# anisanazim/Movie-Recommendation-Engine

Measured on AMD Instinct MI355X. Metric: item embeddings/sec + top-K ANN queries/sec, ML-25M d=256, 1/2/4/8 GPU, higher is better.
Workload: dtype f64 cdf / f32 features / fp4 sign planes (exact integer Hamming); 1 GPU; SYN-25M (ML-25M-shaped: U=162541 M=59047 R=25000095), F=128 H=256 d=256, 2 GCN layers, W=100 L=2 T=10, LSH 512-bit, 10000 queries K=11, rng=numpy (the reference's np.random MT19937 stream generated on device: neighbour ids bit-exact with the reference CPU path); global_items=59047, queries=10000, parallelism=item-shard x1

## Files before the change

movie-recommendation-engine_amd/csrc/mt19937.hip:

```cpp
#include "ps_common.h"

#ifndef PS_MT_DEBUG
#define PS_MT_DEBUG 0
#endif

namespace {

constexpr int MT_N = 624, MT_M = 397;
constexpr int DEG = 19937;
constexpr int CHUNK_LOG2 = 17;
constexpr int64_t CHUNK = (int64_t)1 << CHUNK_LOG2;

struct WinSet { int n; long long first[4]; long long cum[5]; };
struct Wanted { int n; long long lo[4], hi[4]; };
__host__ __device__ __forceinline__ long long win_of(const WinSet &ws, long long q) {
    long long w = ws.first[0] + q;
#pragma unroll
    for (int i = 1; i < 4; ++i)
        if (i < ws.n && q >= ws.cum[i]) w = ws.first[i] + (q - ws.cum[i]);
    return w;
}

__device__ __forceinline__ uint32_t twist(uint32_t u, uint32_t v) {
    const uint32_t y = (u & 0x80000000u) | (v & 0x7fffffffu);
    return (y >> 1) ^ ((v & 1u) ? 0x9908b0dfu : 0u);
}
__device__ __forceinline__ uint32_t temper(uint32_t y) {
    y ^= (y >> 11);
    y ^= (y << 7) & 0x9d2c5680u;
    y ^= (y << 15) & 0xefc60000u;
    y ^= (y >> 18);
    return y;
}

__device__ __forceinline__ void next_block(const uint32_t *o, uint32_t *n, int t) {
    if (t < 227) {
        const uint32_t a = o[t + MT_M] ^ twist(o[t], o[t + 1]);
        const uint32_t b = a ^ twist(o[227 + t], o[228 + t]);
        n[t] = a;
        n[227 + t] = b;
        if (t < 169) n[454 + t] = b ^ twist(o[454 + t], o[455 + t]);
        else if (t == 169) n[623] = b ^ twist(o[623], o[MT_M] ^ twist(o[0], o[1]));
    }
    __syncthreads();
}

template <typename Emit>
__device__ __forceinline__ void next_block_emit(const uint32_t *o, uint32_t *n, int t, Emit emit) {
    if (t < 227) {
        const int t3 = t < 169 ? 454 + t : 622;
        const uint32_t x0 = o[t], x1 = o[t + 1], xm = o[t + MT_M], y0 = o[227 + t], y1 = o[228 + t], z0 = o[t3], z1 = o[t3 + 1];
        const uint32_t l623 = o[623], lm = o[MT_M], l0 = o[0], l1 = o[1];
        const uint32_t a = xm ^ twist(x0, x1);
        const uint32_t b = a ^ twist(y0, y1);
        const uint32_t c = b ^ (t < 169 ? twist(z0, z1) : twist(l623, lm ^ twist(l0, l1)));
        n[t] = a;
        n[227 + t] = b;
        emit(t, a);
        emit(227 + t, b);
        if (t <= 169) {
            const int i3 = t < 169 ? 454 + t : 623;
            n[i3] = c;
            emit(i3, c);
        }
    }
    if (!(PS_MT_DEBUG & 32)) __syncthreads();
}

__device__ __forceinline__ uint32_t untwist(uint32_t tmp) {
    const uint32_t m = (uint32_t)((int32_t)tmp >> 31);
    return __builtin_amdgcn_alignbit(tmp ^ (m & 0x9908b0dfu), tmp, 31);
}

template <typename Emit>
__device__ __forceinline__ void prev_block_emit(const uint32_t *o, uint32_t *p, int t, Emit emit) {
    constexpr uint32_t UP = 0x80000000u, LO = 0x7fffffffu;
    if (t < 227) {
        const int tm = t > 0 ? t - 1 : 0, u = t < 170 ? t : 169;
        const uint32_t a0 = o[t + 395], a1 = o[t + 396], a2 = o[t + 397], b0 = o[t + 168], b1 = o[t + 169], b2 = o[t + 170];
        const uint32_t c0 = o[tm], c1 = o[t], d0 = o[226 + u], d1 = o[227 + u], l622 = o[622], l623 = o[623];
        const uint32_t y397 = untwist(a2 ^ b2), y396 = untwist(a1 ^ b1), y395 = untwist(a0 ^ b0);
        const uint32_t n397 = (y397 & UP) | (y396 & LO);
        const uint32_t n396 = (y396 & UP) | (y395 & LO);
        uint32_t n623 = 0;
        if (t == 0) n623 = (untwist(l623 ^ a1) & UP) | (untwist(l622 ^ a0) & LO);
        const uint32_t ylo = untwist((t > 0 ? c0 : n623) ^ n396);
        const uint32_t nt = (untwist(c1 ^ n397) & UP) | (ylo & LO);
        p[t] = nt;
        p[t + 397] = n397;
        emit(t, nt);
        emit(t + 397, n397);
        if (t < 170) {
            const uint32_t v = (untwist(d1 ^ c1) & UP) | (untwist(d0 ^ (t > 0 ? c0 : n623)) & LO);
            p[227 + t] = v;
            emit(227 + t, v);
        }
    }
    if (!(PS_MT_DEBUG & 32)) __syncthreads();
}

__global__ __launch_bounds__(256) void mt_words_kernel(const uint32_t *state_in, int pos_in, int64_t nwords,
                                                       uint32_t *raw, uint32_t *state_out, int32_t *pos_out) {
    __shared__ uint32_t mt[2][MT_N];
    const int t = threadIdx.x;
    for (int i = t; i < MT_N; i += 256) mt[0][i] = state_in[i];
    __syncthreads();
    int cur = 0, pos = pos_in;
    int64_t done = 0;
    while (done < nwords) {
        if (pos >= MT_N) {
            next_block(mt[cur], mt[cur ^ 1], t);
            cur ^= 1;
            pos = 0;
        }
        const int64_t rem = nwords - done;
        const int take = (MT_N - pos) < rem ? (MT_N - pos) : (int)rem;
        for (int i = t; i < take; i += 256) raw[done + i] = temper(mt[cur][pos + i]);
        pos += take;
        done += take;
    }
    __syncthreads();
    for (int i = t; i < MT_N; i += 256) state_out[i] = mt[cur][i];
    if (t == 0) pos_out[0] = pos;
}

__global__ void mt_pairs_to_double_kernel(double *out, int64_t n) {
    for (int64_t i = (int64_t)blockIdx.x * blockDim.x + threadIdx.x; i < n; i += (int64_t)gridDim.x * blockDim.x) {
        const uint2 w = reinterpret_cast<const uint2 *>(out)[i];
        out[i] = ((double)(w.x >> 5) * 67108864.0 + (double)(w.y >> 6)) * (1.0 / 9007199254740992.0);
    }
}

__global__ __launch_bounds__(256) void mt_prepare_kernel(const uint32_t *state_in, int pos_in, uint32_t *w1,
                                                         uint32_t *word0) {
    __shared__ uint32_t seq[3 * MT_N];
    const int t = threadIdx.x;
    for (int i = t; i < MT_N; i += 256) seq[i] = state_in[i];
    __syncthreads();
    next_block(seq, seq + MT_N, t);
    next_block(seq + MT_N, seq + 2 * MT_N, t);
    for (int i = t; i < MT_N; i += 256) w1[i] = seq[pos_in + 1 + i];
    if (t == 0) word0[0] = seq[pos_in];
}

constexpr int JP = 24;
constexpr int PW = MT_N / JP;
constexpr int SEQ_PAD = 34 * MT_N;
constexpr int XB = 17;
static_assert(SEQ_PAD >= DEG + MT_N && JP * PW == MT_N, "jump geometry");

__device__ __forceinline__ uint32_t load_window_word(const uint32_t *parts, int nparts, int t) {
    uint32_t v = 0;
    for (int p = 0; p < nparts; ++p) v ^= parts[p * MT_N + t];
    return v;
}

__global__ __launch_bounds__(256) void mt_expand_kernel(const uint32_t *src, int nparts, int64_t src_stride, uint32_t *seq) {
    __shared__ uint32_t mt[2][MT_N];
    const int t = threadIdx.x;
    uint32_t *out = seq + (size_t)blockIdx.x * SEQ_PAD;
    for (int i = t; i < MT_N; i += 256) {
        const uint32_t v = load_window_word(src + (size_t)blockIdx.x * src_stride, nparts, i);
        mt[0][i] = v;
        out[i] = v;
    }
    __syncthreads();
    int cur = 0;
    for (int blk = 1; blk < 34; ++blk) {
        uint32_t *dst = out + blk * MT_N;
        next_block_emit(mt[cur], mt[cur ^ 1], t, [&](int i, uint32_t v) { dst[i] = v; });
        cur ^= 1;
    }
}

constexpr int CT = MT_N / 4;
__device__ __forceinline__ void combine_part(const uint32_t *s, const uint32_t *poly_part, uint32_t *dst) {
    __shared__ uint32_t sq[PW * 32 + MT_N + 8];
    __shared__ uint32_t pl[PW];
    const int t = threadIdx.x;
    for (int i = t; i < PW * 32 + MT_N; i += 192) sq[i] = s[i];
    if (t < PW) pl[t] = poly_part[t];
    __syncthreads();
    if (t < CT) {
        uint32_t a0 = 0, a1 = 0, a2 = 0, a3 = 0;
        for (int w = 0; w < PW; ++w) {
            uint32_t bits = pl[w];
            const uint32_t *p = sq + w * 32 + t;
            while (bits) {
                uint32_t v[2][4];
#pragma unroll
                for (int u = 0; u < 2; ++u) {
                    const bool on = bits != 0u;
                    const int bu = on ? __builtin_ctz(bits) : 0;
                    v[u][0] = on ? p[bu] : 0u;
                    v[u][1] = on ? p[bu + CT] : 0u;
                    v[u][2] = on ? p[bu + 2 * CT] : 0u;
                    v[u][3] = on ? p[bu + 3 * CT] : 0u;
                    bits &= bits - 1u;
                }
                a0 ^= v[0][0] ^ v[1][0];
                a1 ^= v[0][1] ^ v[1][1];
                a2 ^= v[0][2] ^ v[1][2];
                a3 ^= v[0][3] ^ v[1][3];
            }
        }
        dst[t] = a0;
        dst[t + CT] = a1;
        dst[t + 2 * CT] = a2;
        dst[t + 3 * CT] = a3;
    }
}

__global__ __launch_bounds__(192) void mt_combine_kernel(const uint32_t *seq, const uint32_t *poly, uint32_t *dst_parts) {
    const int b = blockIdx.x / JP, part = blockIdx.x % JP;
    combine_part(seq + (size_t)b * SEQ_PAD + part * PW * 32, poly + part * PW, dst_parts + ((size_t)b * JP + part) * MT_N);
}

__global__ __launch_bounds__(192) void mt_combine_radix_kernel(const uint32_t *seq, const uint32_t *polys, uint32_t *states,
                                                               int64_t have, int64_t K) {
    const int b = blockIdx.x / JP, part = blockIdx.x % JP;
    const int64_t tgt = (int64_t)(blockIdx.y + 1) * have + b;
    if (tgt >= K) return;
    combine_part(seq + (size_t)b * SEQ_PAD + part * PW * 32, polys + (size_t)blockIdx.y * MT_N + part * PW,
                 states + ((size_t)tgt * JP + part) * MT_N);
}

typedef int v4i_t __attribute__((ext_vector_type(4)));
typedef int v8i_t __attribute__((ext_vector_type(8)));
typedef float v16f_t __attribute__((ext_vector_type(16)));

constexpr int KS_TOTAL = 320;
constexpr int PLW = SEQ_PAD / 32;
constexpr int JT = 20, JG = 10;
constexpr int MF_PLANES = 2;
static_assert(SEQ_PAD % 32 == 0 && JT * 32 >= MT_N && JT == 2 * JG && 32 % MF_PLANES == 0, "plane geometry: two waves x JG lag tiles");

__device__ __forceinline__ uint32_t bits_to_fp4(uint32_t byte) {
    auto four = [](uint32_t n) { return (n | (n << 3) | (n << 6) | (n << 9)) & 0x1111u; };
    return (four(byte & 15u) | (four((byte >> 4) & 15u) << 16)) << 1;
}

__global__ __launch_bounds__(256) void mt_pack_polys_kernel(const uint32_t *__restrict__ polys, int rows, uint4 *__restrict__ polyA) {
    const int idx = blockIdx.x * 256 + threadIdx.x;
    if (idx >= KS_TOTAL * 64) return;
    const int ks = idx >> 6, lane = idx & 63, m = lane & 31, w = 2 * ks + (lane >> 5);
    const uint32_t word = (m < rows && w < MT_N) ? polys[(size_t)m * MT_N + w] : 0u;
    polyA[idx] = make_uint4(bits_to_fp4(word & 255u), bits_to_fp4((word >> 8) & 255u), bits_to_fp4((word >> 16) & 255u),
                            bits_to_fp4(word >> 24));
}

__global__ __launch_bounds__(256) void mt_begin_kernel(const uint32_t *__restrict__ state_in, int pos_in, uint32_t *__restrict__ plain0,
                                                       uint32_t *__restrict__ word0, uint32_t *__restrict__ seq,
                                                       const uint32_t *__restrict__ polys, int nrows, int ngroups, uint4 *__restrict__ polyA,
                                                       WinSet ws) {
    const int t = threadIdx.x;
    if (blockIdx.x < 2) {
        const bool back = blockIdx.x == 1;
        __shared__ uint32_t s3[3 * MT_N];
        __shared__ uint32_t mt[2][MT_N];
        if (state_in != nullptr) {
            for (int i = t; i < MT_N; i += 256) s3[i] = state_in[i];
            __syncthreads();
            next_block(s3, s3 + MT_N, t);
            next_block(s3 + MT_N, s3 + 2 * MT_N, t);
        }
        for (int i = t; i < MT_N; i += 256) {
            const uint32_t v = state_in != nullptr ? s3[pos_in + 1 + i] : plain0[i];
            mt[0][i] = v;
            if (!back) {
                if (state_in != nullptr) plain0[i] = v;
                seq[XB * MT_N + i] = v;
            }
        }
        if (t == 0 && !back && state_in != nullptr) word0[0] = s3[pos_in];
        __syncthreads();
        int cur = 0;
        if (!back) {
            for (int blk = XB + 1; blk < 34; ++blk) {
                uint32_t *dst = seq + blk * MT_N;
                next_block_emit(mt[cur], mt[cur ^ 1], t, [&](int i, uint32_t v) { dst[i] = v; });
                cur ^= 1;
            }
        } else {
            for (int blk = XB - 1; blk >= 0; --blk) {
                uint32_t *dst = seq + blk * MT_N;
                prev_block_emit(mt[cur], mt[cur ^ 1], t, [&](int i, uint32_t v) { dst[i] = v; });
                cur ^= 1;
            }
        }
        return;
    }
    const int64_t idx = (int64_t)(blockIdx.x - 2) * 256 + t;
    if (idx >= (int64_t)ngroups * KS_TOTAL * 64) return;
    const int g = (int)(idx / (KS_TOTAL * 64)), rem = (int)(idx % (KS_TOTAL * 64));
    const int ks = rem >> 6, lane = rem & 63, q = 32 * g + (lane & 31), w = 2 * ks + (lane >> 5);
    const uint32_t word = (q < nrows && w < MT_N) ? polys[(size_t)(win_of(ws, q) - 1) * MT_N + w] : 0u;
    polyA[idx] = make_uint4(bits_to_fp4(word & 255u), bits_to_fp4((word >> 8) & 255u), bits_to_fp4((word >> 16) & 255u),
                            bits_to_fp4(word >> 24));
}

__global__ __launch_bounds__(256) void mt_planes_kernel(const uint32_t *__restrict__ seq, uint32_t *__restrict__ planes) {
    const int lane = threadIdx.x & 63, wv = threadIdx.x >> 6;
    const uint32_t *s = seq + (size_t)blockIdx.y * SEQ_PAD;
    uint32_t *pl = planes + (size_t)blockIdx.y * 32 * PLW;
    for (int grp = blockIdx.x * 4 + wv; grp * 64 < SEQ_PAD; grp += gridDim.x * 4) {
        const int i = grp * 64 + lane;
        const uint32_t word = i < SEQ_PAD ? s[i] : 0u;
#pragma unroll
        for (int b = 0; b < 32; ++b) {
            const uint64_t m = __ballot((word >> b) & 1u);
            if (lane == 0) {
                pl[b * PLW + 2 * grp] = (uint32_t)m;
                if (2 * grp + 1 < PLW) pl[b * PLW + 2 * grp + 1] = (uint32_t)(m >> 32);
            }
        }
    }
}

__device__ __forceinline__ v16f_t bit_mfma(const v4i_t &a, const v4i_t &b, const v16f_t &c) {
    const v8i_t A = {a[0], a[1], a[2], a[3], 0, 0, 0, 0};
    const v8i_t B = {b[0], b[1], b[2], b[3], 0, 0, 0, 0};
    return __builtin_amdgcn_mfma_scale_f32_32x32x64_f8f6f4(A, B, c, 4, 4, 0, 0x7f7f7f7f, 0, 0x7f7f7f7f);
}

__global__ __launch_bounds__(256, 2) void mt_jump_mfma_kernel(const uint32_t *__restrict__ planes, const uint4 *__restrict__ polyA,
                                                              uint16_t *__restrict__ PLp, int nsrc, int parts, int steps, int ngroups) {
    extern __shared__ uint32_t copies[];
    const int tid = threadIdx.x, lane = tid & 63, wv = tid >> 6, pb = wv >> 1, g = wv & 1, n = lane & 31, kb = lane >> 5;
    int item = blockIdx.x;
    const int b0 = (item % (32 / MF_PLANES)) * MF_PLANES; item /= (32 / MF_PLANES);
    const int src = item % nsrc, part = item / nsrc;
    const int ks0 = part * steps, J0 = g * JG;
    const int dmin = 2 * ks0;
    const int CW = 4 * (2 * steps + JT + 1) + 8;
    for (int mm = tid; mm < ((PS_MT_DEBUG & 1) ? 64 : MF_PLANES * CW); mm += 256) {
        const int q = mm / CW, m = mm % CW;
        const uint32_t *pl = planes + ((size_t)(src / ngroups) * 32 + b0 + q) * PLW;
        uint32_t *cp = copies + (size_t)q * 8 * CW;
        const int p0 = 32 * dmin + 8 * m;
        const uint32_t w0 = (p0 >> 5) < PLW ? pl[p0 >> 5] : 0u, w1 = ((p0 + 8) >> 5) < PLW ? pl[(p0 + 8) >> 5] : 0u;
        const uint32_t e0 = bits_to_fp4((w0 >> (p0 & 31)) & 255u), e1 = bits_to_fp4((w1 >> ((p0 + 8) & 31)) & 255u);
        cp[m] = e0;
#pragma unroll
        for (int c = 1; c < 8; ++c) cp[c * CW + m] = __builtin_amdgcn_alignbit(e1, e0, 4 * c);
    }
    __syncthreads();
    const int b = b0 + pb;
    const uint32_t *frag = copies + (size_t)pb * 8 * CW + (n & 7) * CW + 4 * (J0 + kb) + (n >> 3);
    auto load_r = [&](int x) { const uint32_t *q = frag + 4 * x; return v4i_t{(int)q[0], (int)q[1], (int)q[2], (int)q[3]}; };
    const uint4 *pa = polyA + ((size_t)(src % ngroups) * KS_TOTAL + ks0) * 64 + lane;
    auto load_a = [&](v4i_t &dst, int u) {
        const uint4 *ptr = pa + (size_t)u * 64;
        asm volatile("global_load_dwordx4 %0, %1, off" : "=v"(dst) : "v"(ptr) : "memory");
    };

    v16f_t acc[JG];
#pragma unroll
    for (int j = 0; j < JG; ++j)
#pragma unroll
        for (int r = 0; r < 16; ++r) acc[j][r] = 8388608.f;
    constexpr int PF = 5;
    v4i_t R[JG], A[PF];
#pragma unroll
    for (int j = 0; j < JG; ++j) R[j] = load_r(j);
    asm volatile("s_waitcnt vmcnt(0)" ::: "memory");
#pragma unroll
    for (int u = 0; u < PF; ++u) load_a(A[u], u < steps ? u : 0);
    for (int ub = 0; ub < steps; ub += PF) {
#pragma unroll
        for (int uu = 0; uu < PF; ++uu) {
            static_assert(PF == 5, "vmcnt literal below = PF - 1");
            asm volatile("s_waitcnt vmcnt(4)" : "+v"(A[uu]) : : "memory");
            const v4i_t a = A[uu];
#pragma unroll
            for (int jj = 0; jj < JG; ++jj) {
                if (!(PS_MT_DEBUG & 8)) acc[jj] = bit_mfma(a, R[(2 * uu + jj) % JG], acc[jj]);
                else acc[jj][0] += __builtin_bit_cast(float, a[0] ^ R[(2 * uu + jj) % JG][0]);
                if (jj == 1 && !(PS_MT_DEBUG & 64)) {
                    R[(2 * uu) % JG] = load_r(2 * (ub + uu) + JG);
                    R[(2 * uu + 1) % JG] = load_r(2 * (ub + uu) + JG + 1);
                }
            }
            { const int nx = ub + PF + uu; load_a(A[uu], (nx < steps && !(PS_MT_DEBUG & 2)) ? nx : steps - 1); }
            __builtin_amdgcn_sched_barrier(0);
        }
    }
    static_assert(PF == 5, "one operand per ring slot below");
    asm volatile("s_waitcnt vmcnt(0)" : "+v"(A[0]), "+v"(A[1]), "+v"(A[2]), "+v"(A[3]), "+v"(A[4]) : : "memory");
    uint16_t *out = PLp + ((((size_t)part * nsrc + src) * 32 + b) * JT + J0) * 64 + lane;
#pragma unroll
    for (int jj = 0; jj < JG; ++jj) {
        uint32_t bits = 0;
#pragma unroll
        for (int r = 0; r < 16; ++r) {
            const float f = acc[jj][r];
            bits = __builtin_amdgcn_alignbit(__builtin_bit_cast(uint32_t, f), bits, 1);
        }
        bits >>= 16;
        if (!(PS_MT_DEBUG & 4) || bits == 0x12345u) out[jj * 64] = (uint16_t)bits;
    }
}

__global__ __launch_bounds__(256) void mt_jump_reduce_kernel(uint32_t *__restrict__ PLp, int64_t slice_dwords, int parts) {
    const int64_t i = (int64_t)blockIdx.x * 256 + threadIdx.x;
    if (i >= slice_dwords) return;
    uint32_t v = PLp[i];
#pragma unroll 8
    for (int part = 1; part < parts; ++part) v ^= PLp[part * slice_dwords + i];
    PLp[i] = v;
}

__global__ __launch_bounds__(256) void mt_jump_finish_kernel(const uint16_t *__restrict__ PL, int nsrc, int rows, int64_t src_step,
                                                             int64_t m_step, int64_t K, uint32_t *__restrict__ plain) {
    const int64_t idx = (int64_t)blockIdx.x * 256 + threadIdx.x;
    if (idx >= (int64_t)nsrc * rows * MT_N) return;
    const int j = (int)(idx % MT_N), m = (int)((idx / MT_N) % rows), src = (int)(idx / ((int64_t)MT_N * rows));
    const int64_t tgt = src * src_step + (m + 1) * m_step;
    if (tgt >= K) return;
    const int r = (m & 3) | ((m >> 3) << 2), kb = (m >> 2) & 1;
    const uint16_t *p = PL + (((size_t)src * 32) * JT + (j >> 5)) * 64 + 32 * kb + (j & 31);
    uint32_t w = 0;
#pragma unroll
    for (int b = 0; b < 32; ++b) w |= (((uint32_t)p[(size_t)b * JT * 64] >> r) & 1u) << b;
    plain[tgt * MT_N + j] = w;
}

__global__ __launch_bounds__(256) void mt_fold_kernel(const uint32_t *parts, uint32_t *plain) {
    const int i = blockIdx.x * 256 + threadIdx.x;
    if (i >= MT_N) return;
    uint32_t v = 0;
#pragma unroll
    for (int p = 0; p < JP; ++p) v ^= parts[p * MT_N + i];
    plain[i] = v;
}

constexpr int64_t HALF = CHUNK / 2;
template <bool RANGED>
__global__ __launch_bounds__(256) void mt_chunk_kernel(const uint32_t *states, int nparts, int64_t c0, WinSet ws, Wanted wt, int64_t w_lo,
                                                       uint32_t *raw, int64_t key_w, uint32_t *state_out, int pos, int32_t *pos_out,
                                                       const uint32_t *word0) {
    __shared__ uint32_t mt[2][MT_N];
    const int t = threadIdx.x;
    const bool back = blockIdx.y != 0;
    if (blockIdx.x == 0 && !back && t == 0 && key_w >= 1) pos_out[0] = pos;
    if (blockIdx.x == 0 && !back && t == 0 && w_lo == 0) raw[0] = word0[0];
    const int64_t wbase = 1 + (c0 + (blockIdx.x == 0 ? 0 : win_of(ws, blockIdx.x - 1))) * CHUNK;
    int64_t h_lo = back ? wbase - HALF : wbase, h_hi = back ? wbase : wbase + HALF;
    if (h_lo < 1) h_lo = 1;
    int64_t lo = h_hi, hi = h_lo;
#pragma unroll
    for (int i = 0; i < 4; ++i) {
        if (i < wt.n) {
            const int64_t a = wt.lo[i] > h_lo ? wt.lo[i] : h_lo, b = wt.hi[i] < h_hi ? wt.hi[i] : h_hi;
            if (a < b) { lo = a < lo ? a : lo; hi = b > hi ? b : hi; }
        }
    }
    if (lo >= hi) return;
    auto wanted = [&](int64_t w) {
        if (!RANGED) return w >= lo && w < hi;
        bool in = false;
#pragma unroll
        for (int i = 0; i < 4; ++i) in = in || (i < wt.n && w >= wt.lo[i] && w < wt.hi[i]);
        return in && w >= h_lo && w < h_hi;
    };
    auto put = [&](int64_t w0, int i, uint32_t v) {
        const int64_t w = w0 + i;
        if (wanted(w)) {
            raw[w - w_lo] = v;
            if (w >= key_w && w < key_w + MT_N) state_out[w - key_w] = v;
        }
    };
    for (int i = t; i < MT_N; i += 256) {
        const uint32_t v = load_window_word(states + (size_t)blockIdx.x * nparts * MT_N, nparts, i);
        mt[0][i] = v;
        if (!back) put(wbase, i, v);
    }
    __syncthreads();
    auto step = [&](const uint32_t *o, uint32_t *n, int64_t w0) {
        bool whole = !RANGED;
        if (RANGED) {
#pragma unroll
            for (int i = 0; i < 4; ++i) whole = whole || (i < wt.n && w0 >= wt.lo[i] && w0 + MT_N <= wt.hi[i]);
        }
        if (whole && w0 >= (RANGED ? h_lo : lo) && w0 + MT_N <= (RANGED ? h_hi : hi) && (w0 + MT_N <= key_w || w0 >= key_w + MT_N)) {
            uint32_t *dst = raw + (w0 - w_lo);
            if (back) prev_block_emit(o, n, t, [&](int i, uint32_t v) { if (!(PS_MT_DEBUG & 16) || v == 0x12345u) dst[i] = v; });
            else next_block_emit(o, n, t, [&](int i, uint32_t v) { if (!(PS_MT_DEBUG & 16) || v == 0x12345u) dst[i] = v; });
        } else {
            bool any = !RANGED;
            if (RANGED) {
#pragma unroll
                for (int i = 0; i < 4; ++i) any = any || (i < wt.n && w0 < wt.hi[i] && w0 + MT_N > wt.lo[i]);
            }
            if (!any) {
                if (back) prev_block_emit(o, n, t, [&](int, uint32_t) {});
                else next_block_emit(o, n, t, [&](int, uint32_t) {});
            } else {
                if (back) prev_block_emit(o, n, t, [&](int i, uint32_t v) { put(w0, i, v); });
                else next_block_emit(o, n, t, [&](int i, uint32_t v) { put(w0, i, v); });
            }
        }
    };
    if (!back) {
        int64_t w0 = wbase + MT_N;
        for (; w0 + MT_N < hi; w0 += 2 * MT_N) {
            step(mt[0], mt[1], w0);
            step(mt[1], mt[0], w0 + MT_N);
        }
        if (w0 < hi) step(mt[0], mt[1], w0);
    } else {
        int64_t w0 = wbase - MT_N;
        for (; w0 > lo; w0 -= 2 * MT_N) {
            step(mt[0], mt[1], w0);
            step(mt[1], mt[0], w0 - MT_N);
        }
        if (w0 + MT_N > lo) step(mt[0], mt[1], w0);
    }
}

__global__ void mt_raw_to_double_kernel(const uint32_t *raw, int64_t w_lo, int64_t skip, int64_t n, double *out) {
    for (int64_t i = (int64_t)blockIdx.x * blockDim.x + threadIdx.x; i < n; i += (int64_t)gridDim.x * blockDim.x) {
        const int64_t w = 2 * (skip + i) - w_lo;
        const uint32_t a = temper(raw[w]), b = temper(raw[w + 1]);
        out[i] = ((double)(a >> 5) * 67108864.0 + (double)(b >> 6)) * (1.0 / 9007199254740992.0);
    }
}

__global__ void mt_set_pos_kernel(int pos, int32_t *pos_out) { pos_out[0] = pos; }

__global__ void mt_final_state_kernel(const uint32_t *raw, int64_t w_lo, int64_t key_w, int pos, uint32_t *state_out,
                                      int32_t *pos_out) {
    for (int i = threadIdx.x; i < MT_N; i += blockDim.x) state_out[i] = raw[key_w - w_lo + i];
    if (threadIdx.x == 0) pos_out[0] = pos;
}

struct Plan {
    int64_t wa, wb;
    int64_t key_w;
    int pos_out;
    int64_t w_lo, w_hi;
    int64_t c0, c1;
};

Plan make_plan(int pos_in, int64_t skip, int64_t n) {
    Plan p;
    p.wa = 2 * skip;
    p.wb = 2 * (skip + n);
    const int64_t consumed = pos_in + p.wb;
    int64_t q = consumed / MT_N, r = consumed % MT_N;
    if (r == 0 && p.wb > 0) { q -= 1; r = MT_N; }
    p.pos_out = (int)r;
    p.key_w = q * MT_N - pos_in;
    p.w_lo = p.wa;
    if (p.key_w >= 0 && p.key_w < p.w_lo) p.w_lo = p.key_w;
    p.w_hi = p.wb;
    if (p.key_w >= 0 && p.key_w + MT_N > p.w_hi) p.w_hi = p.key_w + MT_N;
    const int64_t first = p.w_lo < 1 ? 1 : p.w_lo, last = p.w_hi - 1;
    p.c0 = (first - 1 + HALF) / CHUNK;
    p.c1 = last >= 1 ? (last - 1 + HALF) / CHUNK : 0;
    if (p.c1 < p.c0) p.c1 = p.c0;
    return p;
}

}

extern "C" int ps_mt19937_chunk_log2(void) { return CHUNK_LOG2; }
extern "C" int ps_mt19937_window_shift(void) { return XB * MT_N; }

static int mt_generate(const uint32_t *state_in, int pos_in, int64_t skip, int64_t n, double *out, uint32_t *raw_out,
                       uint32_t *state_out, int32_t *pos_out, const uint32_t *jump_polys, int jump_levels,
                       const uint32_t *radix_polys, int radix_levels, const uint32_t *window_polys, int n_window,
                       const int64_t *ranges_host, int n_ranges, void *workspace, size_t workspace_bytes, ps_stream_t stream);

extern "C" int ps_mt19937_random_sample(const uint32_t *state_in, int pos_in, int64_t skip, int64_t n, double *out,
                                        uint32_t *state_out, int32_t *pos_out, const uint32_t *jump_polys,
                                        int jump_levels, const uint32_t *radix_polys, int radix_levels,
                                        const uint32_t *window_polys, int n_window, void *workspace,
                                        size_t workspace_bytes, ps_stream_t stream) {
    return mt_generate(state_in, pos_in, skip, n, out, nullptr, state_out, pos_out, jump_polys, jump_levels, radix_polys,
                       radix_levels, window_polys, n_window, nullptr, 0, workspace, workspace_bytes, stream);
}

extern "C" int ps_mt19937_raw_stream(const uint32_t *state_in, int pos_in, int64_t n, uint32_t *raw, uint32_t *state_out,
                                     int32_t *pos_out, const uint32_t *jump_polys, int jump_levels,
                                     const uint32_t *radix_polys, int radix_levels, const uint32_t *window_polys,
                                     int n_window, const int64_t *ranges_host, int n_ranges, void *workspace,
                                     size_t workspace_bytes, ps_stream_t stream) {
    if (!raw || !jump_polys || !workspace || n < (1 << 17) || n_ranges < 0 || (n_ranges > 0 && !ranges_host)) return PS_EINVAL;
    return mt_generate(state_in, pos_in, 0, n, nullptr, raw, state_out, pos_out, jump_polys, jump_levels, radix_polys,
                       radix_levels, window_polys, n_window, ranges_host, n_ranges, workspace, workspace_bytes, stream);
}

extern "C" size_t ps_mt19937_workspace_bytes(int64_t skip, int64_t n) {
    if (n < 0 || skip < 0) return 0;
    const Plan p = make_plan(MT_N, skip, n);
    int64_t K = p.c1 - p.c0 + 3;
    if (K < 128) K = 128;
    const size_t states = ps_align256((size_t)(K + 4) * JP * MT_N * 4);
    const size_t seqs = ps_align256((size_t)(K / 2 + 2) * SEQ_PAD * 4);
    return states + seqs + ps_align256((size_t)(p.w_hi - p.w_lo + 2 * MT_N + CHUNK) * 4) + 4096;
}

static int mt_generate(const uint32_t *state_in, int pos_in, int64_t skip, int64_t n, double *out, uint32_t *raw_out,
                       uint32_t *state_out, int32_t *pos_out, const uint32_t *jump_polys,
                       int jump_levels, const uint32_t *radix_polys, int radix_levels, const uint32_t *window_polys,
                       int n_window, const int64_t *ranges_host, int n_ranges, void *workspace, size_t workspace_bytes,
                       ps_stream_t stream) {
    if (!state_in || !state_out || !pos_out || n < 0 || skip < 0 || pos_in < 0 || pos_in > MT_N) return PS_EINVAL;
    if (n > 0 && !out && !raw_out) return PS_EINVAL;
    hipStream_t st = ps_stream(stream);
    if (n == 0 && skip == 0) {
        if (ps_copy_async(state_out, state_in, MT_N * 4, st) != hipSuccess) return PS_ELAUNCH;
        hipLaunchKernelGGL(mt_set_pos_kernel, dim3(1), dim3(1), 0, st, pos_in, pos_out);
        PS_CHECK_LAUNCH();
        return PS_OK;
    }
    const bool parallel = jump_polys != nullptr && workspace != nullptr && (skip > 0 || n >= (1 << 17));
    if (!parallel) {
        if (skip != 0) return PS_EUNSUPPORTED;
        hipLaunchKernelGGL(mt_words_kernel, dim3(1), dim3(256), 0, st, state_in, pos_in, 2 * n,
                           reinterpret_cast<uint32_t *>(out), state_out, pos_out);
        PS_CHECK_LAUNCH();
        if (n > 0) {
            int64_t grid = ps_cdiv(n, 256);
            if (grid > 8192) grid = 8192;
            hipLaunchKernelGGL(mt_pairs_to_double_kernel, dim3((unsigned)grid), dim3(256), 0, st, out, n);
            PS_CHECK_LAUNCH();
        }
        return PS_OK;
    }
    const Plan p = make_plan(pos_in, skip, n);
    const int64_t K = p.c1 - p.c0 + 1;
    if (workspace_bytes < ps_mt19937_workspace_bytes(skip, n)) return PS_EWORKSPACE;
    if ((p.c1 >> (jump_levels - CHUNK_LOG2)) != 0) return PS_EUNSUPPORTED;
    char *base = ps_ws_base(workspace);
    const size_t WSZ = (size_t)JP * MT_N;
    uint32_t *states = reinterpret_cast<uint32_t *>(base);
    const int64_t Kc = K > 126 ? K : 126;
    uint32_t *tmpA = states + (size_t)(Kc + 1) * WSZ;
    uint32_t *tmpB = tmpA + WSZ;
    uint32_t *word0 = tmpB + WSZ;
    uint32_t *seqs = reinterpret_cast<uint32_t *>(base + ps_align256((size_t)(Kc + 4) * JP * MT_N * 4));
    uint32_t *raw = reinterpret_cast<uint32_t *>(reinterpret_cast<char *>(seqs) + ps_align256((size_t)(Kc / 2 + 2) * SEQ_PAD * 4));
    if (raw_out) {
        if (p.w_lo != 0) return PS_EUNSUPPORTED;
        raw = raw_out;
    }
    WinSet ws;
    Wanted wt;
    wt.n = 1; wt.lo[0] = p.w_lo; wt.hi[0] = p.w_hi;
    ws.n = 1; ws.first[0] = 1; ws.cum[0] = 0; ws.cum[1] = K - 1;
    int64_t Kw = K;
    bool ranged = false;
    if (ranges_host && n_ranges > 0 && n_ranges <= 3 && raw_out && skip == 0 && p.c0 == 0 && window_polys) {
        long long a[4], b[4];
        int m = 0;
        for (int i = 0; i < n_ranges; ++i) {
            const long long lo = ranges_host[2 * i] < 0 ? 0 : ranges_host[2 * i], hi = ranges_host[2 * i + 1] > n ? n : ranges_host[2 * i + 1];
            if (lo < hi) { a[m] = 2 * lo; b[m] = 2 * hi; ++m; }
        }
        if (p.key_w >= 0) { a[m] = p.key_w; b[m] = p.key_w + MT_N; ++m; }
        for (int i = 1; i < m; ++i)
            for (int j = i; j > 0 && a[j] < a[j - 1]; --j) { long long t = a[j]; a[j] = a[j - 1]; a[j - 1] = t; t = b[j]; b[j] = b[j - 1]; b[j - 1] = t; }
        int mm = 0;
        for (int i = 0; i < m; ++i) {
            if (mm > 0 && a[i] <= b[mm - 1]) { if (b[i] > b[mm - 1]) b[mm - 1] = b[i]; }
            else { a[mm] = a[i]; b[mm] = b[i]; ++mm; }
        }
        long long f[4], l[4], maxwin = 0;
        int nw = 0;
        for (int i = 0; i < mm; ++i) {
            const long long a1 = a[i] < 1 ? 1 : a[i];
            if (b[i] <= a1) continue;
            long long clo = (a1 - 1 + HALF) / CHUNK;
            const long long chi = (b[i] - 2 + HALF) / CHUNK;
            if (clo == 0) clo = 1;
            if (chi < clo) continue;
            if (nw > 0 && clo <= l[nw - 1] + 1) { if (chi > l[nw - 1]) l[nw - 1] = chi; }
            else { f[nw] = clo; l[nw] = chi; ++nw; }
            maxwin = l[nw - 1];
        }
        if (mm > 0 && maxwin <= n_window) {
            ranged = true;
            wt.n = mm;
            for (int i = 0; i < mm; ++i) { wt.lo[i] = a[i]; wt.hi[i] = b[i]; }
            ws.n = nw > 0 ? nw : 1;
            ws.cum[0] = 0; ws.cum[1] = 0; ws.first[0] = 1;
            for (int i = 0; i < nw; ++i) { ws.first[i] = f[i]; ws.cum[i + 1] = ws.cum[i] + (l[i] - f[i] + 1); }
            Kw = 1 + ws.cum[ws.n];
        }
    }
    const int64_t nprod = Kw - 1;
    bool plain_states = false;
    uint32_t *plainS = nullptr;
    const int ngroups = (int)((nprod + 31) / 32);
    bool one_round = window_polys != nullptr && (ranged || (K > 32 && K - 1 <= n_window));
    uint32_t *seqM = nullptr, *planes1 = nullptr;
    uint4 *polyAw = nullptr;
    uint16_t *PLw = reinterpret_cast<uint16_t *>(states + WSZ);
    int parts_w = 32;
    {
        double best = 1e30;
        for (int parts = 4; parts <= 32; parts *= 2) {
            const int64_t wgs = (int64_t)ngroups * (32 / MF_PLANES) * parts;
            const double cost = (double)((wgs + 511) / 512) * (KS_TOTAL / parts + 4);
            if (wgs >= 256 && cost < best) { best = cost; parts_w = parts; }
        }
    }
    if (one_round) {
        char *q = reinterpret_cast<char *>(seqs);
        const char *q_end = q + ps_align256((size_t)(Kc / 2 + 2) * SEQ_PAD * 4);
        seqM = reinterpret_cast<uint32_t *>(q);       q += ps_align256((size_t)SEQ_PAD * 4);
        planes1 = reinterpret_cast<uint32_t *>(q);    q += ps_align256((size_t)32 * PLW * 4);
        polyAw = reinterpret_cast<uint4 *>(q);        q += ps_align256((size_t)ngroups * KS_TOTAL * 64 * 16);
        plainS = reinterpret_cast<uint32_t *>(q);     q += ps_align256((size_t)Kw * MT_N * 4);
        one_round = q <= q_end && (size_t)parts_w * ngroups * 32 * JT * 32 <= (size_t)(Kc - 1) * WSZ;
        if (!one_round && ranged) return PS_EWORKSPACE;
    }
    const unsigned pack_blocks = (unsigned)(((int64_t)ngroups * KS_TOTAL * 64 + 255) / 256);
    if (one_round && p.c0 == 0) {
        hipLaunchKernelGGL(mt_begin_kernel, dim3(2 + pack_blocks), dim3(256), 0, st, state_in, pos_in, plainS, word0, seqM, window_polys,
                           (int)nprod, ngroups, polyAw, ws);
        PS_CHECK_LAUNCH();
    } else {
        if (ps_fill_async(tmpA, 0, WSZ * 4, st) != hipSuccess) return PS_ELAUNCH;
        hipLaunchKernelGGL(mt_prepare_kernel, dim3(1), dim3(256), 0, st, state_in, pos_in, tmpA, word0);
        PS_CHECK_LAUNCH();
        uint32_t *cur = tmpA, *nxt = tmpB;
        for (int b = 0; (p.c0 >> b) != 0; ++b) {
            if (!((p.c0 >> b) & 1)) continue;
            hipLaunchKernelGGL(mt_expand_kernel, dim3(1), dim3(256), 0, st, cur, JP, (int64_t)WSZ, seqs);
            PS_CHECK_LAUNCH();
            hipLaunchKernelGGL(mt_combine_kernel, dim3(JP), dim3(192), 0, st, seqs, jump_polys + (size_t)(CHUNK_LOG2 + b) * MT_N, nxt);
            PS_CHECK_LAUNCH();
            uint32_t *t = cur; cur = nxt; nxt = t;
        }
        if (ps_copy_async(states, cur, WSZ * 4, st) != hipSuccess) return PS_ELAUNCH;
        if (one_round) {
            hipLaunchKernelGGL(mt_fold_kernel, dim3(3), dim3(256), 0, st, states, plainS);
            PS_CHECK_LAUNCH();
            hipLaunchKernelGGL(mt_begin_kernel, dim3(2 + pack_blocks), dim3(256), 0, st, (const uint32_t *)nullptr, 0, plainS, word0, seqM,
                               window_polys, (int)nprod, ngroups, polyAw, ws);
            PS_CHECK_LAUNCH();
        }
    }
    if (one_round && nprod == 0) plain_states = true;
    if (one_round && nprod > 0) {
        hipLaunchKernelGGL(mt_planes_kernel, dim3((SEQ_PAD / 64 + 4) / 4, 1), dim3(256), 0, st, seqM, planes1);
        PS_CHECK_LAUNCH();
        const int steps = KS_TOTAL / parts_w;
        const size_t lds = (size_t)MF_PLANES * 8 * (4 * (2 * steps + JT + 1) + 8) * 4;
        hipLaunchKernelGGL(mt_jump_mfma_kernel, dim3((unsigned)(ngroups * (32 / MF_PLANES) * parts_w)), dim3(256), lds, st, planes1, polyAw, PLw, ngroups,
                           parts_w, steps, ngroups);
        PS_CHECK_LAUNCH();
        const int64_t slice = (int64_t)ngroups * 32 * JT * 32;
        hipLaunchKernelGGL(mt_jump_reduce_kernel, dim3((unsigned)ps_cdiv(slice, 256)), dim3(256), 0, st, reinterpret_cast<uint32_t *>(PLw),
                           slice, parts_w);
        PS_CHECK_LAUNCH();
        hipLaunchKernelGGL(mt_jump_finish_kernel, dim3((unsigned)ps_cdiv((int64_t)ngroups * 32 * MT_N, 256)), dim3(256), 0, st, PLw, ngroups,
                           32, (int64_t)32, (int64_t)1, Kw, plainS);
        PS_CHECK_LAUNCH();
        plain_states = true;
    }
    if (!plain_states && radix_polys && radix_levels >= 2 && K > 32 && K <= 1024) {
        const int JA = (int)((K - 1) / 32), nsrcB = JA + 1;
        char *q = reinterpret_cast<char *>(seqs);
        const char *q_end = q + ps_align256((size_t)(K / 2 + 2) * SEQ_PAD * 4);
        uint32_t *seqM = reinterpret_cast<uint32_t *>(q);      q += ps_align256((size_t)nsrcB * SEQ_PAD * 4);
        uint32_t *planes = reinterpret_cast<uint32_t *>(q);    q += ps_align256((size_t)nsrcB * 32 * PLW * 4);
        uint4 *polyA0 = reinterpret_cast<uint4 *>(q);          q += ps_align256((size_t)KS_TOTAL * 64 * 16);
        uint4 *polyA1 = reinterpret_cast<uint4 *>(q);          q += ps_align256((size_t)KS_TOTAL * 64 * 16);
        plainS = reinterpret_cast<uint32_t *>(q);              q += ps_align256((size_t)K * MT_N * 4);
        constexpr int PARTS_A = 32, PARTS_B = 8;
        uint16_t *PLp = reinterpret_cast<uint16_t *>(states + WSZ);
        const bool pl_fits = (size_t)PARTS_B * nsrcB * 32 * JT * 32 <= (size_t)(K - 1) * WSZ && (size_t)PARTS_A * 32 * JT * 32 <= (size_t)(K - 1) * WSZ;
        if (q <= q_end && pl_fits) {
            const unsigned pk = (KS_TOTAL * 64 + 255) / 256;
            hipLaunchKernelGGL(mt_pack_polys_kernel, dim3(pk), dim3(256), 0, st, radix_polys + (size_t)1 * 31 * MT_N, JA, polyA1);
            PS_CHECK_LAUNCH();
            hipLaunchKernelGGL(mt_pack_polys_kernel, dim3(pk), dim3(256), 0, st, radix_polys, 31, polyA0);
            PS_CHECK_LAUNCH();
            hipLaunchKernelGGL(mt_fold_kernel, dim3(3), dim3(256), 0, st, states, plainS);
            PS_CHECK_LAUNCH();
            auto round = [&](int nsrc, const uint4 *polyA, int rows, int parts, int64_t src_step, int64_t m_step) -> int {
                hipLaunchKernelGGL(mt_expand_kernel, dim3((unsigned)nsrc), dim3(256), 0, st, plainS, 1, (int64_t)32 * MT_N, seqM);
                PS_CHECK_LAUNCH();
                hipLaunchKernelGGL(mt_planes_kernel, dim3((SEQ_PAD / 64 + 4) / 4, (unsigned)nsrc), dim3(256), 0, st, seqM, planes);
                PS_CHECK_LAUNCH();
                const int steps = KS_TOTAL / parts;
                const size_t lds = (size_t)MF_PLANES * 8 * (4 * (2 * steps + JT + 1) + 8) * 4;
                hipLaunchKernelGGL(mt_jump_mfma_kernel, dim3((unsigned)(nsrc * (32 / MF_PLANES) * parts)), dim3(256), lds, st, planes, polyA, PLp, nsrc,
                                   parts, steps, 1);
                PS_CHECK_LAUNCH();
                const int64_t total = (int64_t)nsrc * rows * MT_N;
                const int64_t slice = (int64_t)nsrc * 32 * JT * 32;
                hipLaunchKernelGGL(mt_jump_reduce_kernel, dim3((unsigned)ps_cdiv(slice, 256)), dim3(256), 0, st,
                                   reinterpret_cast<uint32_t *>(PLp), slice, parts);
                PS_CHECK_LAUNCH();
                hipLaunchKernelGGL(mt_jump_finish_kernel, dim3((unsigned)ps_cdiv(total, 256)), dim3(256), 0, st, PLp, nsrc, rows, src_step,
                                   m_step, K, plainS);
                PS_CHECK_LAUNCH();
                return PS_OK;
            };
            int rc = round(1, polyA1, JA, PARTS_A, 0, 32);
            if (rc != PS_OK) return rc;
            rc = round(nsrcB, polyA0, 31, PARTS_B, 32, 1);
            if (rc != PS_OK) return rc;
            plain_states = true;
        }
    }
    if (plain_states) {
    } else if (radix_polys && radix_levels > 0) {
        int lvl = 0;
        for (int64_t have = 1; have < K; have *= 32, ++lvl) {
            if (lvl >= radix_levels) return PS_EUNSUPPORTED;
            const int64_t nsrc = (K - have) < have ? (K - have) : have;
            const int64_t jmax = ((K - 1) / have) < 31 ? ((K - 1) / have) : 31;
            hipLaunchKernelGGL(mt_expand_kernel, dim3((unsigned)nsrc), dim3(256), 0, st, states, JP, (int64_t)WSZ, seqs);
            PS_CHECK_LAUNCH();
            hipLaunchKernelGGL(mt_combine_radix_kernel, dim3((unsigned)(nsrc * JP), (unsigned)jmax), dim3(192), 0, st, seqs,
                               radix_polys + (size_t)lvl * 31 * MT_N, states, have, K);
            PS_CHECK_LAUNCH();
        }
    } else {
        for (int m = 0; ((int64_t)1 << m) < K; ++m) {
            const int64_t have = (int64_t)1 << m;
            const int64_t make = (K - have) < have ? (K - have) : have;
            hipLaunchKernelGGL(mt_expand_kernel, dim3((unsigned)make), dim3(256), 0, st, states, JP, (int64_t)WSZ, seqs);
            PS_CHECK_LAUNCH();
            hipLaunchKernelGGL(mt_combine_kernel, dim3((unsigned)(make * JP)), dim3(192), 0, st, seqs,
                               jump_polys + (size_t)(CHUNK_LOG2 + m) * MT_N, states + (size_t)have * WSZ);
            PS_CHECK_LAUNCH();
        }
    }
    const int64_t key_fold = p.key_w >= 1 ? p.key_w : -(int64_t)4 * MT_N;
    if (ranged)
        hipLaunchKernelGGL(mt_chunk_kernel<true>, dim3((unsigned)Kw, 2), dim3(256), 0, st, plain_states ? plainS : states, plain_states ? 1 : JP,
                           p.c0, ws, wt, p.w_lo, raw, key_fold, state_out, p.pos_out, pos_out, word0);
    else
        hipLaunchKernelGGL(mt_chunk_kernel<false>, dim3((unsigned)Kw, 2), dim3(256), 0, st, plain_states ? plainS : states, plain_states ? 1 : JP,
                           p.c0, ws, wt, p.w_lo, raw, key_fold, state_out, p.pos_out, pos_out, word0);
    PS_CHECK_LAUNCH();
    if (n > 0 && !raw_out) {
        int64_t grid = ps_cdiv(n, 256);
        if (grid > 8192) grid = 8192;
        hipLaunchKernelGGL(mt_raw_to_double_kernel, dim3((unsigned)grid), dim3(256), 0, st, raw, p.w_lo, skip, n, out);
        PS_CHECK_LAUNCH();
    }
    if (p.key_w >= 1) {
    } else if (p.key_w == 0) {
        hipLaunchKernelGGL(mt_final_state_kernel, dim3(1), dim3(640), 0, st, raw, p.w_lo, p.key_w, p.pos_out, state_out, pos_out);
        PS_CHECK_LAUNCH();
    } else {
        if (ps_copy_async(state_out, state_in, MT_N * 4, st) != hipSuccess) return PS_ELAUNCH;
        hipLaunchKernelGGL(mt_set_pos_kernel, dim3(1), dim3(1), 0, st, p.pos_out, pos_out);
        PS_CHECK_LAUNCH();
    }
    return PS_OK;
}
```

Baseline: 48.30 million items/s.

## Fuse MT sequence generation with bit-plane transpose inside the begin kernel

The forward and backward MT19937 block chains now keep every generated block in LDS instead of writing the raw sequence to global memory. Spare waves transpose finished 32-word groups into bit planes with DPP/shuffle rounds while the chain waves, raised to high priority, produce the next block. This removes the separate mt_planes_kernel launch and the global round trip of the sequence buffer. In exchange the block grows to 1024 threads with a large LDS footprint, which lowers occupancy for the packing blocks that share the kernel and adds barrier and transpose logic that must stay bit-exact.

```diff
diff --git a/movie-recommendation-engine_amd/csrc/mt19937.hip b/movie-recommendation-engine_amd/csrc/mt19937.hip
--- a/movie-recommendation-engine_amd/csrc/mt19937.hip
+++ b/movie-recommendation-engine_amd/csrc/mt19937.hip
@@ -45,7 +45,7 @@
     __syncthreads();
 }
 
-template <typename Emit>
+template <bool SYNC = true, typename Emit>
 __device__ __forceinline__ void next_block_emit(const uint32_t *o, uint32_t *n, int t, Emit emit) {
     if (t < 227) {
         const int t3 = t < 169 ? 454 + t : 622;
@@ -64,7 +64,7 @@
             emit(i3, c);
         }
     }
-    if (!(PS_MT_DEBUG & 32)) __syncthreads();
+    if (SYNC && !(PS_MT_DEBUG & 32)) __syncthreads();
 }
 
 __device__ __forceinline__ uint32_t untwist(uint32_t tmp) {
@@ -72,7 +72,7 @@
     return __builtin_amdgcn_alignbit(tmp ^ (m & 0x9908b0dfu), tmp, 31);
 }
 
-template <typename Emit>
+template <bool SYNC = true, typename Emit>
 __device__ __forceinline__ void prev_block_emit(const uint32_t *o, uint32_t *p, int t, Emit emit) {
     constexpr uint32_t UP = 0x80000000u, LO = 0x7fffffffu;
     if (t < 227) {
@@ -96,7 +96,7 @@
             emit(227 + t, v);
         }
     }
-    if (!(PS_MT_DEBUG & 32)) __syncthreads();
+    if (SYNC && !(PS_MT_DEBUG & 32)) __syncthreads();
 }
 
 __global__ __launch_bounds__(256) void mt_words_kernel(const uint32_t *state_in, int pos_in, int64_t nwords,
@@ -249,48 +249,93 @@
                             bits_to_fp4(word >> 24));
 }
 
-__global__ __launch_bounds__(256) void mt_begin_kernel(const uint32_t *__restrict__ state_in, int pos_in, uint32_t *__restrict__ plain0,
-                                                       uint32_t *__restrict__ word0, uint32_t *__restrict__ seq,
+template <int J, uint32_t M>
+__device__ __forceinline__ uint32_t transpose_round(uint32_t x, int lane) {
+    int y;
+    if (J == 16) y = __shfl_xor((int)x, 16, 64);
+    else if (J == 8) y = __builtin_amdgcn_update_dpp(0, (int)x, 0x128, 0xf, 0xf, true);
+    else if (J == 4) y = __builtin_amdgcn_update_dpp(0, __builtin_amdgcn_update_dpp(0, (int)x, 0x141, 0xf, 0xf, true), 0x1B, 0xf, 0xf, true);
+    else y = __builtin_amdgcn_update_dpp(0, (int)x, J == 2 ? 0x4E : 0xB1, 0xf, 0xf, true);
+    const uint32_t u = (uint32_t)y;
+    return (lane & J) ? (((u >> J) & M) | (x & ~M)) : ((x & M) | ((u & M) << J));
+}
+__device__ __forceinline__ uint32_t transpose32(uint32_t x, int lane) {
+    x = transpose_round<16, 0x0000ffffu>(x, lane);
+    x = transpose_round<8, 0x00ff00ffu>(x, lane);
+    x = transpose_round<4, 0x0f0f0f0fu>(x, lane);
+    x = transpose_round<2, 0x33333333u>(x, lane);
+    return transpose_round<1, 0x55555555u>(x, lane);
+}
+constexpr int G_SPLIT = (XB * MT_N + 31) / 32;
+
+constexpr int BEGIN_THREADS = 1024, BEGIN_CHAIN_WAVES = 4;
+__device__ __forceinline__ void lds_barrier() {
+    __builtin_amdgcn_fence(__ATOMIC_RELEASE, "workgroup", "local");
+    __builtin_amdgcn_s_barrier();
+    __builtin_amdgcn_fence(__ATOMIC_ACQUIRE, "workgroup", "local");
+}
+__global__ __launch_bounds__(BEGIN_THREADS) void mt_begin_kernel(const uint32_t *__restrict__ state_in, int pos_in, uint32_t *__restrict__ plain0,
+                                                       uint32_t *__restrict__ word0, uint32_t *__restrict__ planes,
                                                        const uint32_t *__restrict__ polys, int nrows, int ngroups, uint4 *__restrict__ polyA,
                                                        WinSet ws) {
     const int t = threadIdx.x;
     if (blockIdx.x < 2) {
         const bool back = blockIdx.x == 1;
         __shared__ uint32_t s3[3 * MT_N];
-        __shared__ uint32_t mt[2][MT_N];
+        __shared__ uint32_t all[(XB + 1) * MT_N];
+        static_assert(34 - XB <= XB + 1, "both chains fit the block store");
+        const int lane = t & 63, wv = t >> 6, li = lane & 31, lh = lane >> 5;
+        const int wbase = back ? 0 : XB * MT_N;
         if (state_in != nullptr) {
-            for (int i = t; i < MT_N; i += 256) s3[i] = state_in[i];
+            for (int i = t; i < MT_N; i += BEGIN_THREADS) s3[i] = state_in[i];
             __syncthreads();
             next_block(s3, s3 + MT_N, t);
             next_block(s3 + MT_N, s3 + 2 * MT_N, t);
         }
-        for (int i = t; i < MT_N; i += 256) {
+        uint32_t *win = all + (XB * MT_N - wbase);
+        for (int i = t; i < MT_N; i += BEGIN_THREADS) {
             const uint32_t v = state_in != nullptr ? s3[pos_in + 1 + i] : plain0[i];
-            mt[0][i] = v;
-            if (!back) {
-                if (state_in != nullptr) plain0[i] = v;
-                seq[XB * MT_N + i] = v;
-            }
+            win[i] = v;
+            if (!back && state_in != nullptr) plain0[i] = v;
         }
         if (t == 0 && !back && state_in != nullptr) word0[0] = s3[pos_in];
         __syncthreads();
-        int cur = 0;
+        if (wv < BEGIN_CHAIN_WAVES) __builtin_amdgcn_s_setprio(3);
+        auto put_pairs = [&](int g0, int np, int w0) __attribute__((always_inline)) {
+            for (int p = wv - w0; p >= 0 && p < np; p += BEGIN_THREADS / 64 - w0) {
+                const int g = back ? g0 - 2 * p - lh : g0 + 2 * p + lh;
+                const bool ok = g < PLW;
+                const uint32_t x = transpose32(ok ? all[32 * g + li - wbase] : 0u, lane);
+                if (ok) planes[li * PLW + g] = x;
+            }
+        };
         if (!back) {
+            int cg = G_SPLIT;
             for (int blk = XB + 1; blk < 34; ++blk) {
-                uint32_t *dst = seq + blk * MT_N;
-                next_block_emit(mt[cur], mt[cur ^ 1], t, [&](int i, uint32_t v) { dst[i] = v; });
-                cur ^= 1;
+                const uint32_t *o = all + (blk - 1 - XB) * MT_N;
+                next_block_emit<false>(o, all + (blk - XB) * MT_N, t, [](int, uint32_t) {});
+                const int np = ((blk * MT_N) / 32 - cg) / 2;
+                put_pairs(cg, np, BEGIN_CHAIN_WAVES);
+                cg += 2 * np;
+                lds_barrier();
             }
+            put_pairs(cg, (PLW - cg + 1) / 2, 0);
         } else {
+            int cg = G_SPLIT;
             for (int blk = XB - 1; blk >= 0; --blk) {
-                uint32_t *dst = seq + blk * MT_N;
-                prev_block_emit(mt[cur], mt[cur ^ 1], t, [&](int i, uint32_t v) { dst[i] = v; });
-                cur ^= 1;
+                const uint32_t *o = all + (blk + 1) * MT_N;
+                prev_block_emit<false>(o, all + blk * MT_N, t, [](int, uint32_t) {});
+                const int np = (cg - ((blk + 1) * MT_N + 31) / 32) / 2;
+                put_pairs(cg - 1, np, BEGIN_CHAIN_WAVES);
+                cg -= 2 * np;
+                lds_barrier();
             }
+            static_assert(G_SPLIT % 2 == 0, "the backward chain's groups are whole pairs");
+            put_pairs(cg - 1, cg / 2, 0);
         }
         return;
     }
-    const int64_t idx = (int64_t)(blockIdx.x - 2) * 256 + t;
+    const int64_t idx = (int64_t)(blockIdx.x - 2) * BEGIN_THREADS + t;
     if (idx >= (int64_t)ngroups * KS_TOTAL * 64) return;
     const int g = (int)(idx / (KS_TOTAL * 64)), rem = (int)(idx % (KS_TOTAL * 64));
     const int ks = rem >> 6, lane = rem & 63, q = 32 * g + (lane & 31), w = 2 * ks + (lane >> 5);
@@ -695,7 +740,7 @@
     uint32_t *plainS = nullptr;
     const int ngroups = (int)((nprod + 31) / 32);
     bool one_round = window_polys != nullptr && (ranged || (K > 32 && K - 1 <= n_window));
-    uint32_t *seqM = nullptr, *planes1 = nullptr;
+    uint32_t *planes1 = nullptr;
     uint4 *polyAw = nullptr;
     uint16_t *PLw = reinterpret_cast<uint16_t *>(states + WSZ);
     int parts_w = 32;
@@ -710,16 +755,16 @@
     if (one_round) {
         char *q = reinterpret_cast<char *>(seqs);
         const char *q_end = q + ps_align256((size_t)(Kc / 2 + 2) * SEQ_PAD * 4);
-        seqM = reinterpret_cast<uint32_t *>(q);       q += ps_align256((size_t)SEQ_PAD * 4);
+        q += ps_align256((size_t)SEQ_PAD * 4);
         planes1 = reinterpret_cast<uint32_t *>(q);    q += ps_align256((size_t)32 * PLW * 4);
         polyAw = reinterpret_cast<uint4 *>(q);        q += ps_align256((size_t)ngroups * KS_TOTAL * 64 * 16);
         plainS = reinterpret_cast<uint32_t *>(q);     q += ps_align256((size_t)Kw * MT_N * 4);
         one_round = q <= q_end && (size_t)parts_w * ngroups * 32 * JT * 32 <= (size_t)(Kc - 1) * WSZ;
         if (!one_round && ranged) return PS_EWORKSPACE;
     }
-    const unsigned pack_blocks = (unsigned)(((int64_t)ngroups * KS_TOTAL * 64 + 255) / 256);
+    const unsigned pack_blocks = (unsigned)(((int64_t)ngroups * KS_TOTAL * 64 + BEGIN_THREADS - 1) / BEGIN_THREADS);
     if (one_round && p.c0 == 0) {
-        hipLaunchKernelGGL(mt_begin_kernel, dim3(2 + pack_blocks), dim3(256), 0, st, state_in, pos_in, plainS, word0, seqM, window_polys,
+        hipLaunchKernelGGL(mt_begin_kernel, dim3(2 + pack_blocks), dim3(BEGIN_THREADS), 0, st, state_in, pos_in, plainS, word0, planes1, window_polys,
                            (int)nprod, ngroups, polyAw, ws);
         PS_CHECK_LAUNCH();
     } else {
@@ -739,15 +784,13 @@
         if (one_round) {
             hipLaunchKernelGGL(mt_fold_kernel, dim3(3), dim3(256), 0, st, states, plainS);
             PS_CHECK_LAUNCH();
-            hipLaunchKernelGGL(mt_begin_kernel, dim3(2 + pack_blocks), dim3(256), 0, st, (const uint32_t *)nullptr, 0, plainS, word0, seqM,
+            hipLaunchKernelGGL(mt_begin_kernel, dim3(2 + pack_blocks), dim3(BEGIN_THREADS), 0, st, (const uint32_t *)nullptr, 0, plainS, word0, planes1,
                                window_polys, (int)nprod, ngroups, polyAw, ws);
             PS_CHECK_LAUNCH();
         }
     }
     if (one_round && nprod == 0) plain_states = true;
     if (one_round && nprod > 0) {
-        hipLaunchKernelGGL(mt_planes_kernel, dim3((SEQ_PAD / 64 + 4) / 4, 1), dim3(256), 0, st, seqM, planes1);
-        PS_CHECK_LAUNCH();
         const int steps = KS_TOTAL / parts_w;
         const size_t lds = (size_t)MF_PLANES * 8 * (4 * (2 * steps + JT + 1) + 8) * 4;
         hipLaunchKernelGGL(mt_jump_mfma_kernel, dim3((unsigned)(ngroups * (32 / MF_PLANES) * parts_w)), dim3(256), lds, st, planes1, polyAw, PLw, ngroups,
```

Measured after the change: 48.24 million items/s. No clear change (-0.1%).
